# jianzhnie/ScaleRL

Hardware: NVIDIA H100
Metric: learner_frames_per_sec (higher is better)
Workload: dtype bf16

## Files before the change

### scalerl_b200/csrc/common.cuh

```cuda
#pragma once
#include <cuda_runtime.h>
#include <cuda_bf16.h>
#include <stdint.h>
#include "wgmma.cuh"

#define SRL_DEVINL __device__ __forceinline__

#ifndef SRL_SPIN_LIMIT
#define SRL_SPIN_LIMIT (1u << 24)
#endif

namespace srl {

SRL_DEVINL uint32_t smem_u32(const void* p) { return static_cast<uint32_t>(__cvta_generic_to_shared(p)); }

SRL_DEVINL void mbar_init(uint64_t* bar, uint32_t count) {
  asm volatile("mbarrier.init.shared::cta.b64 [%0], %1;" ::"r"(smem_u32(bar)), "r"(count) : "memory");
}
SRL_DEVINL void mbar_fence_init() { asm volatile("fence.mbarrier_init.release.cluster;" ::: "memory"); }
SRL_DEVINL void mbar_arrive(uint64_t* bar) {
  asm volatile("{\n\t.reg .b64 st;\n\tmbarrier.arrive.shared::cta.b64 st, [%0];\n\t}" ::"r"(smem_u32(bar)) : "memory");
}
SRL_DEVINL void mbar_arrive_expect_tx(uint64_t* bar, uint32_t bytes) {
  asm volatile("{\n\t.reg .b64 st;\n\tmbarrier.arrive.expect_tx.shared::cta.b64 st, [%0], %1;\n\t}" ::"r"(smem_u32(bar)), "r"(bytes)
// ... 111 lines not shown

SRL_DEVINL uint64_t make_smem_desc(uint32_t saddr, uint32_t lbo_bytes, uint32_t sbo_bytes) {
  uint64_t d = 0;
  d |= (uint64_t)((saddr & 0x3FFFF) >> 4);
  d |= (uint64_t)((lbo_bytes >> 4) & 0x3FFF) << 16;
  d |= (uint64_t)((sbo_bytes >> 4) & 0x3FFF) << 32;
  d |= (uint64_t)1 << 62;
  return d;
}
SRL_DEVINL uint64_t make_smem_desc_sw64(uint32_t saddr, uint32_t lbo_bytes, uint32_t sbo_bytes) {
  return (make_smem_desc(saddr, lbo_bytes, sbo_bytes) & ~((uint64_t)3 << 62)) | ((uint64_t)2 << 62);
}

SRL_DEVINL uint32_t swz128(uint32_t row, uint32_t chunk) { return row * 128u + ((chunk ^ (row & 7u)) << 4); }
SRL_DEVINL uint32_t swz64(uint32_t row, uint32_t chunk) { return row * 64u + ((chunk ^ ((row >> 1) & 3u)) << 4); }

SRL_DEVINL uint32_t pack_bf16x2(float lo, float hi) {
  __nv_bfloat162 v = __floats2bfloat162_rn(lo, hi);
  return *reinterpret_cast<uint32_t*>(&v);
}
SRL_DEVINL float bf16_lo(uint32_t v) { return __uint_as_float(v << 16); }
SRL_DEVINL float bf16_hi(uint32_t v) { return __uint_as_float(v & 0xFFFF0000u); }

SRL_DEVINL void red_add_v4(float* addr, float a, float b, float c, float d) {
  asm volatile("red.global.add.v4.f32 [%0], {%1, %2, %3, %4};" ::"l"(addr), "f"(a), "f"(b), "f"(c), "f"(d) : "memory");
}
SRL_DEVINL void red_add_16(float* dst, const float (&v)[16], float scale = 1.0f) {
#pragma unroll
  for (int j = 0; j < 16; j += 4) red_add_v4(dst + j, v[j] * scale, v[j + 1] * scale, v[j + 2] * scale, v[j + 3] * scale);
}

SRL_DEVINL int ld_action(const int64_t* p, int A) {
  const long long a = __ldg(reinterpret_cast<const long long*>(p));
  return a < 0 ? 0 : (a >= A ? A - 1 : (int)a);
}

SRL_DEVINL float warp_sum(float v) {
#pragma unroll
  for (int o = 16; o > 0; o >>= 1) v += __shfl_xor_sync(0xffffffffu, v, o);
  return v;
}

SRL_DEVINL bool take_ticket(float* scratch) {
  __threadfence();
  return atomicAdd(reinterpret_cast<unsigned*>(scratch), 1u) == gridDim.x - 1;
}
// ... 3 lines not shown
```

### scalerl_b200/csrc/encoder.cu

```cuda
#include "encoder_problems.cuh"
#include "tma_problems.cuh"
#include "res_problems.cuh"
#include "enc_fused.cuh"
#include "kernels.h"
#include <stdio.h>
#include <stdlib.h>

namespace srl {

constexpr int PACK_BLOCKS_FK = 256, PACK_BLOCKS_FD = 256, PACK_BLOCKS_CONV = 288;
SRL_DEVINL void pack_store(bf16* __restrict__ out, bf16* __restrict__ out_lo, int64_t i, float v) {
  const bf16 hi = __float2bfloat16_rn(v);
  out[i] = hi;
  if (out_lo) out_lo[i] = __float2bfloat16_rn(v - __bfloat162float(hi));
}
SRL_DEVINL void pack_store2(bf16* __restrict__ out, bf16* __restrict__ out_lo, int64_t i, float v0, float v1) {
  const bf16 h0 = __float2bfloat16_rn(v0), h1 = __float2bfloat16_rn(v1);
  *reinterpret_cast<uint32_t*>(out + i) = pack_bf16x2(v0, v1);
  if (out_lo) *reinterpret_cast<uint32_t*>(out_lo + i) = pack_bf16x2(v0 - __bfloat162float(h0), v1 - __bfloat162float(h1));
}
__global__ void __launch_bounds__(256) pack_weights_kernel(ParamPtrs p, bf16* __restrict__ out, bf16* __restrict__ out_lo, int skip_w1k) {
  pdl_wait(2);
  __shared__ __align__(16) float tile[64 * 99];
  const int t = threadIdx.x, b = blockIdx.x;
// ... 324 lines not shown
    static_assert(TFcFwd::SPLITS == FC_SPLITS, "split count");
    S.b(PS_FC_FWD);
    if (sp) SRL_TRY((igemm_tma_launch<TFcFwd, 1>(q, dim3(cdiv(frames, 128), 8 * FC_SPLITS), st)));
    else SRL_TRY((igemm_tma_launch<TFcFwd, 0>(q, dim3(cdiv(frames, 128), 8 * FC_SPLITS), st)));
    S.e(PS_FC_FWD); }
  return cudaSuccess;
}

cudaError_t encoder_backward(int frames, const EncoderBuffers& buf, const ParamPtrs& g, const TmaMaps& maps, int mode,
                             const StepStreams& S, BwdParts parts, bool a3t_done) {
  if (frames <= 0) return cudaSuccess;
  if ((mode != 0 && mode != 1) || !maps.valid) return cudaErrorInvalidValue;
  const int sp = mode;
  if (sp && !buf.lo.wpack) return cudaErrorInvalidValue;
  const bool do_fc = parts & BWD_FC, do_conv = parts & BWD_CONV;
  const cudaStream_t st = S.main, s1 = S.lane(LANE_FC_WGRAD), s2 = S.lane(LANE_CONV3_WGRAD), s3 = S.lane(LANE_CONV2_WGRAD);
  if (do_fc) {
    SRL_TRY(S.fork(LANE_FC_WGRAD));
    { const bool native = !sp && buf.a3t != nullptr;
      S.b(PS_FC_WGRAD);
      if (native) {
        if (!a3t_done) SRL_TRY(launch_a3_transpose(buf.hi.a3, buf.a3t, frames, s1));
        TFcWgradN::Params q{maps.hi.dhm64, maps.a3tm64, g.wf, g.bf, frames};
        SRL_TRY((igemm_tma_launch<TFcWgradN, 0>(q, dim3(1, 4 * (TFcWgradN::NCT + 1)), s1)));
      } else {
        TFcWgrad::Params q{maps.hi.dhm64, maps.hi.a3m64, maps.lo.dhm64, maps.lo.a3m64, g.wf, g.bf, frames};
        if (sp) SRL_TRY((igemm_tma_launch<TFcWgrad, 1>(q, dim3(1, 4 * 50), s1))); else SRL_TRY((igemm_tma_launch<TFcWgrad, 0>(q, dim3(1, 4 * 50), s1)));
      }
      S.e(PS_FC_WGRAD); }
    { TFcDgrad::Params q{maps.hi.dhm128, maps.hi.wfd, maps.lo.dhm128, maps.lo.wfd, buf.hi.a3, buf.hi.da3, buf.lo.da3, frames};
      S.b(PS_FC_DGRAD);
      if (sp) SRL_TRY((igemm_tma_launch<TFcDgrad, 1>(q, dim3(cdiv(frames, 128), 49), st))); else SRL_TRY((igemm_tma_launch<TFcDgrad, 0>(q, dim3(cdiv(frames, 128), 49), st)));
      S.e(PS_FC_DGRAD); }
    if (!do_conv) SRL_TRY(S.join(LANE_FC_WGRAD));
  }
  if (!do_conv) return cudaSuccess;
  SRL_TRY(S.fork(LANE_CONV3_WGRAD));
  float* part3 = buf.wgrad_part;
  float* part2 = part3 + (size_t)WG_PART_CTAS * WSP_W3;
  float* part1 = part2 + (size_t)WG_PART_CTAS * WSP_W2;
  int n3 = 0, n2 = 0, n1 = 0;
  { RConv3Wgrad::Params q{maps.hi.a2_w, maps.hi.da3g_b, maps.lo.a2_w, maps.lo.da3g_b, part3, frames * 81, 0};
    S.b(PS_CONV3_WGRAD); SRL_TRY(res_wgrad_launch<RConv3Wgrad>(q, side_wgrad_ctas(), s2, &n3, sp)); S.e(PS_CONV3_WGRAD); }
  if (!S.collapsed) SRL_TRY(launch_wgrad_reduce<WgradReduce3>(part3, n3, g.w3, g.b3, s2));
  { RConv3Dgrad::Params q{maps.hi.da3g_w, maps.hi.w3d, maps.lo.da3g_w, maps.lo.w3d, buf.hi.a2, buf.hi.da2, buf.lo.da2, frames};
    S.b(PS_CONV3_DGRAD); SRL_TRY(res_fwd_launch<RConv3Dgrad>(q, cdiv(frames * 81, 128), bwd_ctas(), st, sp)); S.e(PS_CONV3_DGRAD); }
  SRL_TRY(S.fork(LANE_CONV2_WGRAD));
// ... 22 lines not shown
```

### scalerl_b200/csrc/igemm_res.cuh

```cuda
#pragma once
#include "igemm_tma.cuh"

namespace srl {

constexpr int RES_THREADS = 384;
constexpr int RES_PRODUCER_REGS = 40, RES_CONSUMER_REGS = 232;
constexpr int RES_MAX_TAPS = 10;


template <int N, int ROWB, class F>
SRL_DEVINL void wg_acc_stage_bf16(const float (&d)[2][N / 2], uint8_t* buf, int wt, int bar, F f) {
  static_assert(ROWB % 16 == 0 && ROWB >= 2 * N, "16-byte aligned rows that hold N bf16");
  const int w = wt >> 5, l = wt & 31;
  named_bar(bar, 128);
#pragma unroll
  for (int h = 0; h < 2; ++h)
#pragma unroll
    for (int i = 0; i < N / 2; i += 2) {
      const int row = 64 * h + 16 * w + (l >> 2) + 8 * ((i >> 1) & 1), col = 8 * (i >> 2) + 2 * (l & 3);
      *reinterpret_cast<uint32_t*>(buf + row * ROWB + col * 2) = pack_bf16x2(f(col, d[h][i]), f(col + 1, d[h][i + 1]));
    }
  named_bar(bar, 128);
}
template <class P, int SPLIT>
struct ResFwdCfg {
  static constexpr int ALO = (SPLIT && P::A_LO) ? 1 : 0;
  static constexpr int WIN_BYTES = ((P::WROWS * 128 + 1023) / 1024) * 1024;
  static constexpr int IN_HI_BYTES = P::NWIN * WIN_BYTES;
  static constexpr int IN_BYTES = IN_HI_BYTES * (1 + ALO);
  static constexpr int W_HI_BYTES = P::NT * P::BN * 128;
  static constexpr int W_BYTES = W_HI_BYTES * (1 + SPLIT);
  static constexpr bool TILE_EPI = P::TILE_ROWB > 0 && !SPLIT;
  static constexpr int TILE_IMG_BYTES = 128 * P::TILE_ROWB > WG_IMG_BYTES ? 128 * P::TILE_ROWB : WG_IMG_BYTES;
  static constexpr bool IMG1 = !TILE_EPI && W_BYTES + IN_BYTES + 2 * WG_IMG_BYTES + 1024 + 256 > 232448;
  static constexpr int IMG_BYTES = TILE_EPI ? TILE_IMG_BYTES : IMG1 ? WG_IMG_BYTES / 2 : WG_IMG_BYTES;
  static constexpr int FIT = fit_stages(SPLIT ? P::SPLIT_STAGES : P::STAGES, W_BYTES + 2 * IMG_BYTES + 1024 + 256, IN_BYTES);
  static constexpr int STAGES = FIT > 1 ? FIT & ~1 : 1;
  static constexpr int SMEM_BYTES = W_BYTES + STAGES * IN_BYTES + 2 * IMG_BYTES + 1024 + 256;
  static_assert(SMEM_BYTES <= 232448, "shared memory budget (227 KB)");
  static_assert(W_BYTES % 1024 == 0, "weight block alignment");
  static_assert(P::BN == 32 || P::BN == 64 || P::BN == 128, "MMA N");
};

template <class P, int SPLIT>
__global__ void __launch_bounds__(RES_THREADS, 1) res_fwd_kernel(const __grid_constant__ typename P::Params p) {
  using C = ResFwdCfg<P, SPLIT>;
// ... 362 lines not shown
```

### scalerl_b200/csrc/igemm_tma.cuh

```cuda
#pragma once
#include <cuda.h>
#include "common.cuh"
#include "kernels.h"

namespace srl {

SRL_DEVINL void tma_prefetch_desc(const CUtensorMap* m) {
  asm volatile("prefetch.tensormap [%0];" ::"l"(reinterpret_cast<uint64_t>(m)) : "memory");
}
SRL_DEVINL void tma_load_2d(void* dst, const CUtensorMap* m, uint64_t* bar, int c0, int c1) {
  asm volatile("cp.async.bulk.tensor.2d.shared::cluster.global.mbarrier::complete_tx::bytes [%0], [%1, {%3, %4}], [%2];"
               ::"r"(smem_u32(dst)), "l"(reinterpret_cast<uint64_t>(m)), "r"(smem_u32(bar)), "r"(c0), "r"(c1) : "memory");
}
SRL_DEVINL void tma_load_3d(void* dst, const CUtensorMap* m, uint64_t* bar, int c0, int c1, int c2) {
  asm volatile("cp.async.bulk.tensor.3d.shared::cluster.global.mbarrier::complete_tx::bytes [%0], [%1, {%3, %4, %5}], [%2];"
               ::"r"(smem_u32(dst)), "l"(reinterpret_cast<uint64_t>(m)), "r"(smem_u32(bar)), "r"(c0), "r"(c1), "r"(c2) : "memory");
}
SRL_DEVINL void tma_load_4d(void* dst, const CUtensorMap* m, uint64_t* bar, int c0, int c1, int c2, int c3) {
  asm volatile("cp.async.bulk.tensor.4d.shared::cluster.global.mbarrier::complete_tx::bytes [%0], [%1, {%3, %4, %5, %6}], [%2];"
               ::"r"(smem_u32(dst)), "l"(reinterpret_cast<uint64_t>(m)), "r"(smem_u32(bar)), "r"(c0), "r"(c1), "r"(c2), "r"(c3)
               : "memory");
}
SRL_DEVINL void tma_load_5d(void* dst, const CUtensorMap* m, uint64_t* bar, int c0, int c1, int c2, int c3, int c4) {
  asm volatile("cp.async.bulk.tensor.5d.shared::cluster.global.mbarrier::complete_tx::bytes [%0], [%1, {%3, %4, %5, %6, %7}], [%2];"
               ::"r"(smem_u32(dst)), "l"(reinterpret_cast<uint64_t>(m)), "r"(smem_u32(bar)), "r"(c0), "r"(c1), "r"(c2), "r"(c3), "r"(c4)
               : "memory");
}

constexpr int IGT_THREADS = 288;

template <class P, int SPLIT = 0>
struct TmaCfg {
  static constexpr int KROWS = P::A_MN ? P::KROWS : 64;
  static constexpr int A_BYTES = P::A_MN ? 2 * KROWS * 128 : 128 * 128;
  static constexpr int B_BLOCKS = (P::BN + 63) / 64;
  static constexpr int B_BYTES = P::B_MN ? B_BLOCKS * KROWS * 128 : P::BN * 128;
  static constexpr int HALF_BYTES = A_BYTES + B_BYTES;
  static constexpr int STAGE_BYTES = HALF_BYTES * (1 + SPLIT);
  static constexpr int NB = P::BN / 2;
  static constexpr int STAGES = fit_stages(P::STAGES, 2 * WG_IMG_BYTES + 1024 + 256, STAGE_BYTES);
  static constexpr int SMEM_BYTES = STAGES * STAGE_BYTES + 2 * WG_IMG_BYTES + 1024 + 256;
  static_assert(SMEM_BYTES <= 232448, "shared memory budget (227 KB)");
  static_assert(NB == 32 || NB == 64 || NB == 128, "MMA N per warpgroup");
  static constexpr int MMAS = P::A_MN ? KROWS / 16 : 4;
  static_assert(A_BYTES % 1024 == 0 && B_BYTES % 1024 == 0, "operand tiles must keep 1024 B alignment (SWIZZLE_128B atoms)");
  static_assert(P::A_MN == P::B_MN, "mixed majors are not used");
  static_assert(KROWS % 16 == 0, "contraction rows per stage must be a multiple of MMA K = 16");
};

template <class P, int SPLIT>
SRL_DEVINL void igt_epilogue(const typename P::Params& p, int tm, int ty, int row, int c0, float (&v)[16]) {
  if constexpr (SPLIT) P::template epilogue16<1>(p, tm, ty, row, c0, v); else P::epilogue16(p, tm, ty, row, c0, v);
}
template <class P, int SPLIT>
SRL_DEVINL void igt_epilogue(const typename P::Params& p, int tm, int ty, int row, int c0, float (&v)[16], const uint4 (&pre)[2]) {
  if constexpr (SPLIT) P::template epilogue16<1>(p, tm, ty, row, c0, v, pre); else P::epilogue16(p, tm, ty, row, c0, v, pre);
}

template <class P, int SPLIT = 0>
__global__ void __launch_bounds__(IGT_THREADS) igemm_tma_kernel(const __grid_constant__ typename P::Params p) {
  using C = TmaCfg<P, SPLIT>;
  extern __shared__ uint8_t smem_raw[];
  uint8_t* smem = reinterpret_cast<uint8_t*>((reinterpret_cast<uintptr_t>(smem_raw) + 1023) & ~uintptr_t(1023));
  float* img = reinterpret_cast<float*>(smem + C::STAGES * C::STAGE_BYTES);
  uint64_t* bars = reinterpret_cast<uint64_t*>(smem + C::STAGES * C::STAGE_BYTES + 2 * WG_IMG_BYTES);
  uint64_t* full = bars;
  uint64_t* empty = bars + C::STAGES;

  const int tid = threadIdx.x;
  const int warp = tid >> 5;
  const int tm = blockIdx.x, ty = blockIdx.y;
  const int nkb = P::num_kblocks(p, tm, ty);

  if constexpr (P::ZERO_INIT) {
    if (P::zero_cta(ty)) {
      uint4* z = reinterpret_cast<uint4*>(smem);
      for (int i = tid; i < C::STAGES * C::STAGE_BYTES / 16; i += IGT_THREADS) z[i] = make_uint4(0, 0, 0, 0);
    }
    __syncthreads();
    for (int s = 0; s < C::STAGES; ++s) P::init_smem(p, tm, ty, smem + s * C::STAGE_BYTES, tid);
    fence_proxy_async_smem();
  }
  if (warp == 8 && (tid & 31) == 0) {
    for (int s = 0; s < C::STAGES; ++s) { mbar_init(&full[s], 1); mbar_init(&empty[s], 8); }
    mbar_fence_init();
    P::prefetch(p);
  }
  __syncthreads();
  pdl_wait(P::KID);
  if (tid == 256) pdl_launch();

  if (warp == 8) {
    const uint32_t leader = elect_one_sync();
    for (int kb = 0; kb < nkb; ++kb) {
      const int s = kb % C::STAGES;
      mbar_wait(&empty[s], ((kb / C::STAGES) & 1) ^ 1);
      if (leader) {
        uint8_t* sA = smem + s * C::STAGE_BYTES;
// ... 27 lines not shown
      wg_fence();
#pragma unroll
      for (int k = 0; k < C::MMAS; ++k) {
        const uint64_t ad = ad0 + (uint64_t)(k * ASTEP), bd = bd0 + (uint64_t)(k * BSTEP);
        wg_mma128<NB, P::A_MN ? 1 : 0, P::B_MN ? 1 : 0>(acc, ad, A_HI, bd, (kb | k) != 0);
        if constexpr (SPLIT) {
          wg_mma128<NB, P::A_MN ? 1 : 0, P::B_MN ? 1 : 0>(acc, ad, A_HI, bd + (uint64_t)(C::HALF_BYTES / 16), 1);
          wg_mma128<NB, P::A_MN ? 1 : 0, P::B_MN ? 1 : 0>(acc, ad + (uint64_t)(C::HALF_BYTES / 16), A_HI, bd, 1);
        }
      }
      wg_commit();
      if constexpr (C::STAGES > 1) {
        wg_wait_prev();
        __syncwarp();
        if (kb > 0 && (tid & 31) == 0) mbar_arrive(&empty[(kb - 1) % C::STAGES]);
      } else {
        wg_wait_all();
        __syncwarp();
        if ((tid & 31) == 0) mbar_arrive(&empty[s]);
      }
    }
    wg_wait_all();
    wg_fence_regs(acc[0]); wg_fence_regs(acc[1]);
    float* my_img = img + g * (WG_IMG_BYTES / 4);
#pragma unroll
    for (int c = 0; c < NB / 16; ++c) {
      float v[16];
      wg_acc_row16<NB>(acc, c, my_img, wt, 2 + g, v);
      if constexpr (P::PREFETCH) igt_epilogue<P, SPLIT>(p, tm, ty, wt, g * NB + c * 16, v, pre[c]);
      else igt_epilogue<P, SPLIT>(p, tm, ty, wt, g * NB + c * 16, v);
    }
  }
}

template <class P, int SPLIT = 0>
cudaError_t igemm_tma_launch(const typename P::Params& p, dim3 grid, cudaStream_t stream) {
  using C = TmaCfg<P, SPLIT>;
  if (grid.x == 0 || grid.y == 0) return cudaSuccess;
  static PerDeviceOnce once;
  { cudaError_t e = ensure_max_dynamic_smem(once, igemm_tma_kernel<P, SPLIT>, C::SMEM_BYTES); if (e != cudaSuccess) return e; }
  return launch_chain(igemm_tma_kernel<P, SPLIT>, grid, dim3(IGT_THREADS), C::SMEM_BYTES, stream, p);
}

}
```

### scalerl_b200/csrc/lstm.cu

```cuda
#include <new>
#include "tma_problems.cuh"
#include "kernels.h"
#include "errors.h"
#include "../../include/scalerl_b200.h"

namespace srl {

struct LGemmK {
  static constexpr int KID = 34;
  static constexpr bool PREFETCH = false;
  static constexpr int BN = 64, STAGES = 4, KROWS = 64;
  static constexpr bool A_MN = false, B_MN = false, ZERO_INIT = false;
  struct Params { SRL_TMAP a; SRL_TMAP b; float* C; int M, nkb, ldc, a_row0, c_row0; };
  SRL_DEVINL static void prefetch(const Params& p) { tma_prefetch_desc(&p.a); tma_prefetch_desc(&p.b); }
  SRL_DEVINL static int num_kblocks(const Params& p, int, int) { return p.nkb; }
  SRL_DEVINL static void issue(const Params& p, int tm, int ty, int kb, uint8_t* sA, uint8_t* sB, uint64_t* bar) {
    mbar_arrive_expect_tx(bar, 128 * 128 + 64 * 128);
    tma_load_2d(sA, &p.a, bar, kb * 64, p.a_row0 + tm * 128);
    tma_load_2d(sB, &p.b, bar, kb * 64, ty * 64);
  }
  SRL_DEVINL static void epilogue16(const Params& p, int tm, int ty, int row, int c0, float (&v)[16]) {
    const int m = tm * 128 + row;
    if (m >= p.M) return;
    float4* o = reinterpret_cast<float4*>(p.C + (size_t)(p.c_row0 + m) * p.ldc + ty * 64 + c0);
#pragma unroll
    for (int j = 0; j < 4; ++j) o[j] = make_float4(v[4 * j], v[4 * j + 1], v[4 * j + 2], v[4 * j + 3]);
  }
};
struct LGemmMN {
  static constexpr int KID = 35;
  static constexpr bool PREFETCH = false;
  static constexpr int BN = 64, STAGES = 4, KROWS = 64;
  static constexpr bool A_MN = true, B_MN = true, ZERO_INIT = false;
  struct Params { SRL_TMAP a; SRL_TMAP b; float* C; int R, ldc; };
  SRL_DEVINL static void prefetch(const Params& p) { tma_prefetch_desc(&p.a); tma_prefetch_desc(&p.b); }
  SRL_DEVINL static int num_kblocks(const Params& p, int, int) { return (p.R + 63) >> 6; }
  SRL_DEVINL static void init_smem(const Params&, int, int, uint8_t*, int, int) {}
  SRL_DEVINL static void issue(const Params& p, int tm, int ty, int kb, uint8_t* sA, uint8_t* sB, uint64_t* bar) {
    mbar_arrive_expect_tx(bar, 3 * 64 * 128);
    tma_load_2d(sA, &p.a, bar, tm * 128, kb * 64);
    tma_load_2d(sA + KROWS * 128, &p.a, bar, tm * 128 + 64, kb * 64);
    tma_load_2d(sB, &p.b, bar, ty * 64, kb * 64);
  }
  SRL_DEVINL static void epilogue16(const Params& p, int tm, int ty, int row, int c0, float (&v)[16]) {
    float4* o = reinterpret_cast<float4*>(p.C + (size_t)(tm * 128 + row) * p.ldc + ty * 64 + c0);
#pragma unroll
    for (int j = 0; j < 4; ++j) o[j] = make_float4(v[4 * j], v[4 * j + 1], v[4 * j + 2], v[4 * j + 3]);
  }
};

SRL_DEVINL float sigmoidf_(float x) { return 1.0f / (1.0f + expf(-x)); }

__global__ void lstm_pad_bf16_kernel(const float* __restrict__ x, int rows, int H, int Hp, __nv_bfloat16* __restrict__ out) {
  const int64_t i = (int64_t)blockIdx.x * blockDim.x + threadIdx.x;
  if (i >= (int64_t)rows * Hp) return;
  const int r = (int)(i / Hp), j = (int)(i - (int64_t)r * Hp);
// ... 658 lines not shown
```

### scalerl_b200/csrc/res_problems.cuh

```cuda
#pragma once
#include "igemm_res.cuh"
#include "encoder_problems.cuh"

namespace srl {

template <int SPLIT>
SRL_DEVINL void store_act16(bf16* hi, bf16* lo, size_t elem_off, const float (&v)[16]) {
  store_bf16x16(hi + elem_off, v);
  if constexpr (SPLIT) {
    float r[16];
#pragma unroll
    for (int j = 0; j < 16; ++j) r[j] = v[j] - __bfloat162float(__float2bfloat16_rn(v[j]));
    store_bf16x16(lo + elem_off, r);
  }
}

struct RConv1Fwd {
  static constexpr int KID = 11;
  static constexpr int BN = 32, NT = 4, NWIN = 1, WROWS = 128 + 22, STAGES = 4, SPLIT_STAGES = 4;
  static constexpr bool A_LO = false;
  struct Params { SRL_TMAP in0; SRL_TMAP w; SRL_TMAP w_lo; const float* bias; bf16* out; bf16* out_lo; int NF; int NFS; };
  static constexpr bool W_AFTER_WAIT = true;
  SRL_DEVINL static void prefetch(const Params& p) { tma_prefetch_desc(&p.in0); tma_prefetch_desc(&p.w); }
  SRL_DEVINL static int num_tiles(const Params& p) { return (p.NF * 441 + 127) >> 7; }
  SRL_DEVINL static constexpr int tap_win(int) { return 0; }
  SRL_DEVINL static constexpr int tap_shift(int j) { return (j >> 1) * 21 + (j & 1); }
  SRL_DEVINL static void load_windows(const Params& p, int t, uint8_t* dst, int, uint64_t* bar, bool) { tma_load_2d(dst, &p.in0, bar, 0, t * 128); }
  SRL_DEVINL static void prefetch16(const Params&, int, int, int, uint4 (&)[2]) {}
  static constexpr int TILE_ROWB = 80;
  SRL_DEVINL static void prefetch_tile(const Params&, int, int, uint4 (&)[BN / 16][2]) {}
  SRL_DEVINL static void epilogue_tile(const Params& p, int t, int wt, const float (&acc)[2][BN / 2], uint8_t* img, int bar,
                                       const uint4 (&)[BN / 16][2]) {
    wg_acc_stage_bf16<BN, TILE_ROWB>(acc, img, wt, bar, [&](int c, float v) { return fmaxf(fmaf(v, 1.0f / 255.0f, __ldg(p.bias + c)), 0.f); });
#pragma unroll
    for (int s = 0; s < 4; ++s) {
      const int e = s * 128 + wt, q = e >> 2, k = e & 3;
      const int Q = t * 128 + q, n = Q / 441, r = Q - n * 441, oh = r / 21, ow = r - oh * 21;
      if (n >= p.NF || oh >= 20 || ow >= 20) continue;
      const size_t prow = (size_t)(oh & 1) * p.NFS * 100 + (size_t)n * 100 + (oh >> 1) * 10 + (ow >> 1);
      *reinterpret_cast<uint4*>(p.out + prow * 64 + (ow & 1) * 32 + k * 8) = *reinterpret_cast<const uint4*>(img + q * TILE_ROWB + k * 16);
    }
  }
  template <int SPLIT>
  SRL_DEVINL static void epilogue16(const Params& p, int t, int row, int c0, float (&v)[16], const uint4 (&)[2]) {
    const int Q = t * 128 + row, n = Q / 441, r = Q - n * 441, oh = r / 21, ow = r - oh * 21;
    if (n >= p.NF || oh >= 20 || ow >= 20) return;
#pragma unroll
    for (int j = 0; j < 16; ++j) v[j] = fmaxf(fmaf(v[j], 1.0f / 255.0f, __ldg(p.bias + c0 + j)), 0.f);
    const size_t prow = (size_t)(oh & 1) * p.NFS * 100 + (size_t)n * 100 + (oh >> 1) * 10 + (ow >> 1);
    store_act16<SPLIT>(p.out, p.out_lo, prow * 64 + (ow & 1) * 32 + c0, v);
  }
};

struct RConv2Fwd {
  static constexpr int KID = 12;
  static constexpr bool W_AFTER_WAIT = false;
// ... 73 lines not shown
  static constexpr bool W_AFTER_WAIT = false;
  static constexpr int BN = 128, NT = 4, NWIN = 1, WROWS = 128 + 11, STAGES = 3, SPLIT_STAGES = 2;
  static constexpr bool A_LO = true;
  struct Params { SRL_TMAP in0; SRL_TMAP w; SRL_TMAP in0_lo; SRL_TMAP w_lo; const bf16* act; bf16* dx; bf16* dx_lo; int NB; int NF; };
  SRL_DEVINL static void prefetch(const Params& p) { tma_prefetch_desc(&p.in0); tma_prefetch_desc(&p.w); }
  SRL_DEVINL static int num_tiles(const Params& p) { return (p.NB * 100 + 127) >> 7; }
  SRL_DEVINL static constexpr int tap_win(int) { return 0; }
  SRL_DEVINL static constexpr int tap_shift(int j) { return 11 - ((j >> 1) * 10 + (j & 1)); }
  SRL_DEVINL static void load_windows(const Params& p, int t, uint8_t* dst, int, uint64_t* bar, bool lo) { tma_load_2d(dst, lo ? &p.in0_lo : &p.in0, bar, 0, t * 128 - 11); }
  SRL_DEVINL static void prefetch16(const Params& p, int t, int row, int c0, uint4 (&m)[2]) {
    const int Q = t * 128 + row, cls = c0 >> 5, c = c0 & 31;
    if (Q < p.NB * 100) ld_mask16(p.act + ((size_t)(cls >> 1) * p.NF * 100 + Q) * 64 + (cls & 1) * 32 + c, m);
  }
  static constexpr int TILE_ROWB = 272;
  SRL_DEVINL static void prefetch_tile(const Params& p, int t, int wt, uint4 (&m)[BN / 16][2]) {
#pragma unroll
    for (int s = 0; s < 16; ++s) {
      const int e = s * 128 + wt, ph = e >> 10, Q = t * 128 + ((e >> 3) & 127);
      if (Q < p.NB * 100) m[s >> 1][s & 1] = ldg16(p.act + ((size_t)ph * p.NF * 100 + Q) * 64 + (e & 7) * 8);
    }
  }
  SRL_DEVINL static void epilogue_tile(const Params& p, int t, int wt, const float (&acc)[2][BN / 2], uint8_t* img, int bar,
                                       const uint4 (&m)[BN / 16][2]) {
    wg_acc_stage_bf16<BN, TILE_ROWB>(acc, img, wt, bar, [](int, float v) { return v; });
#pragma unroll
    for (int s = 0; s < 16; ++s) {
      const int e = s * 128 + wt, ph = e >> 10, q = (e >> 3) & 127, k = e & 7;
      const int Q = t * 128 + q, n = Q / 100, r = Q - n * 100, i = r / 10, j = r - i * 10;
      if (n >= p.NB) continue;
      const uint4 x = *reinterpret_cast<const uint4*>(img + q * TILE_ROWB + ph * 128 + k * 16), mk = m[s >> 1][s & 1];
      *reinterpret_cast<uint4*>(p.dx + ((size_t)n * 441 + (2 * i + ph) * 21 + 2 * j) * 32 + k * 8) =
          make_uint4(relu_mask_bf16x2(x.x, mk.x), relu_mask_bf16x2(x.y, mk.y), relu_mask_bf16x2(x.z, mk.z), relu_mask_bf16x2(x.w, mk.w));
    }
  }
  template <int SPLIT>
  SRL_DEVINL static void epilogue16(const Params& p, int t, int row, int c0, float (&v)[16], const uint4 (&m)[2]) {
    const int Q = t * 128 + row, n = Q / 100, r = Q - n * 100, i = r / 10, j = r - i * 10;
    if (n >= p.NB) return;
    const int cls = c0 >> 5, c = c0 & 31, ph = cls >> 1, pw = cls & 1;
    relu_mask16_pre(m, v);
    store_act16<SPLIT>(p.dx, p.dx_lo, ((size_t)n * 441 + (2 * i + ph) * 21 + 2 * j + pw) * 32 + c, v);
  }
};

struct RConv3Wgrad {
  static constexpr int KID = 21;
  static constexpr int NBLK = 9, CWG = 3, NWIN = 1, WROWS = 128 + 20, STAGES = 3, SPLIT_STAGES = 2;
// ... 45 lines not shown
```

### scalerl_b200/csrc/tma_problems.cuh

```cuda
#pragma once
#include "igemm_tma.cuh"
#include "encoder_problems.cuh"

namespace srl {

#define SRL_TMAP alignas(64) CUtensorMap

struct TFcFwd {
  static constexpr int KID = 31;
  static constexpr bool PREFETCH = false;
  static constexpr int BN = 64, STAGES = 4, SPLITS = 4;
  static constexpr bool A_MN = false, B_MN = false, ZERO_INIT = false;
  static constexpr int KROWS = 64;
  struct Params { SRL_TMAP a3m; SRL_TMAP w; SRL_TMAP a3m_lo; SRL_TMAP w_lo; float* out; int M; };
  SRL_DEVINL static void prefetch(const Params& p) { tma_prefetch_desc(&p.a3m); tma_prefetch_desc(&p.w); }
  SRL_DEVINL static int kb_begin(int split) { return (49 * split) / SPLITS; }
  SRL_DEVINL static void issue_split(const Params& p, int tm, int ty, int kb, uint8_t* st, int a_bytes, int half, uint64_t* bar) {
    const int k = (kb_begin(ty % SPLITS) + kb) * 64;
    mbar_arrive_expect_tx(bar, 2 * (128 * 128 + 64 * 128));
    tma_load_2d(st, &p.a3m, bar, k, tm * 128);
    tma_load_2d(st + a_bytes, &p.w, bar, k, (ty / SPLITS) * 64);
    tma_load_2d(st + half, &p.a3m_lo, bar, k, tm * 128);
    tma_load_2d(st + half + a_bytes, &p.w_lo, bar, k, (ty / SPLITS) * 64);
  }
  template <int SPLIT>
  SRL_DEVINL static void epilogue16(const Params& p, int tm, int ty, int row, int c0, float (&v)[16]) { epilogue16(p, tm, ty, row, c0, v); }
  SRL_DEVINL static int num_kblocks(const Params&, int, int ty) { const int sp = ty % SPLITS; return kb_begin(sp + 1) - kb_begin(sp); }
  SRL_DEVINL static void issue(const Params& p, int tm, int ty, int kb, uint8_t* sA, uint8_t* sB, uint64_t* bar) {
    const int k = (kb_begin(ty % SPLITS) + kb) * 64;
    mbar_arrive_expect_tx(bar, 128 * 128 + 64 * 128);
    tma_load_2d(sA, &p.a3m, bar, k, tm * 128);
    tma_load_2d(sB, &p.w, bar, k, (ty / SPLITS) * 64);
  }
  SRL_DEVINL static void epilogue16(const Params& p, int tm, int ty, int row, int c0, float (&v)[16]) {
    const int m = tm * 128 + row;
    if (m >= p.M) return;
    float4* o = reinterpret_cast<float4*>(p.out + ((size_t)(ty % SPLITS) * p.M + m) * 512 + (ty / SPLITS) * 64 + c0);
#pragma unroll
    for (int j = 0; j < 4; ++j) o[j] = make_float4(v[4 * j], v[4 * j + 1], v[4 * j + 2], v[4 * j + 3]);
  }
};

struct TFcDgrad {
  static constexpr int KID = 32;
  static constexpr bool PREFETCH = true;
  static constexpr int BN = 64, STAGES = 4;
  static constexpr bool A_MN = false, B_MN = false, ZERO_INIT = false;
  static constexpr int KROWS = 64;
  struct Params { SRL_TMAP dhm; SRL_TMAP w; SRL_TMAP dhm_lo; SRL_TMAP w_lo; const bf16* a3; bf16* da3; bf16* da3_lo; int M; };
  SRL_DEVINL static void prefetch(const Params& p) { tma_prefetch_desc(&p.dhm); tma_prefetch_desc(&p.w); }
  SRL_DEVINL static int num_kblocks(const Params&, int, int) { return 8; }
  SRL_DEVINL static void issue_split(const Params& p, int tm, int ty, int kb, uint8_t* st, int a_bytes, int half, uint64_t* bar) {
    mbar_arrive_expect_tx(bar, 2 * (128 * 128 + 64 * 128));
    tma_load_2d(st, &p.dhm, bar, kb * 64, tm * 128);
    tma_load_2d(st + a_bytes, &p.w, bar, kb * 64, ty * 64);
    tma_load_2d(st + half, &p.dhm_lo, bar, kb * 64, tm * 128);
    tma_load_2d(st + half + a_bytes, &p.w_lo, bar, kb * 64, ty * 64);
  }
  SRL_DEVINL static void issue(const Params& p, int tm, int ty, int kb, uint8_t* sA, uint8_t* sB, uint64_t* bar) {
    mbar_arrive_expect_tx(bar, 128 * 128 + 64 * 128);
    tma_load_2d(sA, &p.dhm, bar, kb * 64, tm * 128);
    tma_load_2d(sB, &p.w, bar, kb * 64, ty * 64);
  }
  SRL_DEVINL static void prefetch16(const Params& p, int tm, int ty, int row, int c0, uint4 (&mk)[2]) {
    const int m = tm * 128 + row;
    if (m < p.M) ld_mask16(p.a3 + (size_t)m * 3136 + ty * 64 + c0, mk);
  }
  SRL_DEVINL static void epilogue16(const Params& p, int tm, int ty, int row, int c0, float (&v)[16], const uint4 (&mk)[2]) {
    epilogue16<0>(p, tm, ty, row, c0, v, mk);
  }
// ... 2 lines not shown
    const int m = tm * 128 + row;
    if (m >= p.M) return;
    relu_mask16_pre(mk, v);
    const size_t o = ((size_t)m * 81 + (ty / 7) * 9 + ty % 7) * 64 + c0;
    store_bf16x16(p.da3 + o, v);
    if constexpr (SPLIT) {
      float r[16];
#pragma unroll
      for (int j = 0; j < 16; ++j) r[j] = v[j] - __bfloat162float(__float2bfloat16_rn(v[j]));
      store_bf16x16(p.da3_lo + o, r);
    }
  }
};

SRL_DEVINL void fill_ones(uint8_t* dst, int bytes, int tid) {
  uint4* q = reinterpret_cast<uint4*>(dst);
  for (int i = tid; i < bytes / 16; i += IGT_THREADS) q[i] = make_uint4(0x3F803F80u, 0x3F803F80u, 0x3F803F80u, 0x3F803F80u);
}

struct TFcWgrad {
  static constexpr int KID = 33;
  static constexpr bool PREFETCH = false;
  static constexpr int BN = 64, STAGES = 4, KROWS = 64;
  static constexpr bool A_MN = true, B_MN = true, ZERO_INIT = true;
  struct Params { SRL_TMAP dhm; SRL_TMAP a3m; SRL_TMAP dhm_lo; SRL_TMAP a3m_lo; float* dw; float* db; int M; };
  SRL_DEVINL static void prefetch(const Params& p) { tma_prefetch_desc(&p.dhm); tma_prefetch_desc(&p.a3m); }
  SRL_DEVINL static void issue_split(const Params& p, int, int ty, int kb, uint8_t* st, int a_bytes, int half, uint64_t* bar) {
    const int hw = ty >> 2, j0 = (ty & 3) * 128;
    mbar_arrive_expect_tx(bar, (hw < 49 ? 6 : 4) * 64 * 128);
    tma_load_2d(st, &p.dhm, bar, j0, kb * 64);
    tma_load_2d(st + KROWS * 128, &p.dhm, bar, j0 + 64, kb * 64);
    tma_load_2d(st + half, &p.dhm_lo, bar, j0, kb * 64);
    tma_load_2d(st + half + KROWS * 128, &p.dhm_lo, bar, j0 + 64, kb * 64);
    if (hw < 49) {
      tma_load_2d(st + a_bytes, &p.a3m, bar, hw * 64, kb * 64);
      tma_load_2d(st + half + a_bytes, &p.a3m_lo, bar, hw * 64, kb * 64);
    }
  }
  template <int SPLIT>
  SRL_DEVINL static void epilogue16(const Params& p, int tm, int ty, int row, int c0, float (&v)[16]) { epilogue16(p, tm, ty, row, c0, v); }
  SRL_DEVINL static bool zero_cta(int) { return true; }
  SRL_DEVINL static int num_kblocks(const Params& p, int, int) { return (p.M + 63) >> 6; }
  SRL_DEVINL static void init_smem(const Params&, int, int ty, uint8_t* stage, int tid) {
    if ((ty >> 2) == 49) fill_ones(stage + 2 * KROWS * 128, KROWS * 128, tid);
  }
  SRL_DEVINL static void issue(const Params& p, int, int ty, int kb, uint8_t* sA, uint8_t* sB, uint64_t* bar) {
    const int hw = ty >> 2, j0 = (ty & 3) * 128;
    mbar_arrive_expect_tx(bar, (hw < 49 ? 3 : 2) * 64 * 128);
    tma_load_2d(sA, &p.dhm, bar, j0, kb * 64);
    tma_load_2d(sA + KROWS * 128, &p.dhm, bar, j0 + 64, kb * 64);
    if (hw < 49) tma_load_2d(sB, &p.a3m, bar, hw * 64, kb * 64);
  }
  SRL_DEVINL static void epilogue16(const Params& p, int, int ty, int row, int c0, float (&v)[16]) {
    const int j = (ty & 3) * 128 + row, hw = ty >> 2;
    if (hw < 49) {
#pragma unroll
      for (int jj = 0; jj < 16; ++jj) p.dw[(size_t)j * 3136 + (c0 + jj) * 49 + hw] = v[jj];
    } else if (c0 == 0) {
      p.db[j] = v[0];
    }
  }
};

struct TFcWgradN {
  static constexpr int KID = 36;
  static constexpr bool PREFETCH = false;
  static constexpr int BN = 256, STAGES = 4, KROWS = 64, NCT = 13;
  static constexpr bool A_MN = true, B_MN = true, ZERO_INIT = true;
  struct Params { SRL_TMAP dhm; SRL_TMAP a3tm; float* dw; float* db; int M; };
  SRL_DEVINL static void prefetch(const Params& p) { tma_prefetch_desc(&p.dhm); tma_prefetch_desc(&p.a3tm); }
  SRL_DEVINL static bool zero_cta(int ty) { return (ty >> 2) == NCT; }
  SRL_DEVINL static int num_kblocks(const Params& p, int, int) { return (p.M + 63) >> 6; }
  SRL_DEVINL static void init_smem(const Params&, int, int ty, uint8_t* stage, int tid) {
    if ((ty >> 2) == NCT) fill_ones(stage + 2 * KROWS * 128, KROWS * 128, tid);
  }
  SRL_DEVINL static void issue(const Params& p, int, int ty, int kb, uint8_t* sA, uint8_t* sB, uint64_t* bar) {
    const int ct = ty >> 2, j0 = (ty & 3) * 128;
    const int nb = ct < NCT ? (ct == NCT - 1 ? 1 : 4) : 0;
    mbar_arrive_expect_tx(bar, (2 + nb) * 64 * 128);
    tma_load_2d(sA, &p.dhm, bar, j0, kb * 64);
    tma_load_2d(sA + KROWS * 128, &p.dhm, bar, j0 + 64, kb * 64);
    for (int q = 0; q < nb; ++q) tma_load_2d(sB + q * KROWS * 128, &p.a3tm, bar, ct * 256 + q * 64, kb * 64);
  }
  SRL_DEVINL static void epilogue16(const Params& p, int, int ty, int row, int c0, float (&v)[16]) {
    const int j = (ty & 3) * 128 + row, ct = ty >> 2, col = ct * 256 + c0;
    if (ct < NCT) {
      if (col < 3136) {
        float4* d = reinterpret_cast<float4*>(p.dw + (size_t)j * 3136 + col);
#pragma unroll
        for (int q = 0; q < 4; ++q) d[q] = make_float4(v[4 * q], v[4 * q + 1], v[4 * q + 2], v[4 * q + 3]);
      }
    } else if (c0 == 0) {
      p.db[j] = v[0];
    }
  }
};

}
```

Measured before the change: 2.483 million.

## Fold FC wgrad bias into last column tile and stage epilogue through ring

```diff
diff --git a/scalerl_b200/csrc/common.cuh b/scalerl_b200/csrc/common.cuh
--- a/scalerl_b200/csrc/common.cuh
+++ b/scalerl_b200/csrc/common.cuh
@@ -157,6 +157,24 @@
 SRL_DEVINL float bf16_lo(uint32_t v) { return __uint_as_float(v << 16); }
 SRL_DEVINL float bf16_hi(uint32_t v) { return __uint_as_float(v & 0xFFFF0000u); }
 
+template <int N, int ROWB, class T, class F>
+SRL_DEVINL void wg_acc_stage(const float (&d)[2][N / 2], uint8_t* buf, int wt, int bar, F f) {
+  static_assert(ROWB % 16 == 0 && ROWB >= (int)sizeof(T) * N, "16-byte aligned rows that hold N values");
+  const int w = wt >> 5, l = wt & 31;
+  named_bar(bar, 128);
+#pragma unroll
+  for (int h = 0; h < 2; ++h)
+#pragma unroll
+    for (int i = 0; i < N / 2; i += 2) {
+      const int row = 64 * h + 16 * w + (l >> 2) + 8 * ((i >> 1) & 1), col = 8 * (i >> 2) + 2 * (l & 3);
+      if constexpr (sizeof(T) == 2)
+        *reinterpret_cast<uint32_t*>(buf + row * ROWB + col * 2) = pack_bf16x2(f(col, d[h][i]), f(col + 1, d[h][i + 1]));
+      else
+        *reinterpret_cast<float2*>(buf + row * ROWB + col * 4) = make_float2(f(col, d[h][i]), f(col + 1, d[h][i + 1]));
+    }
+  named_bar(bar, 128);
+}
+
 SRL_DEVINL void red_add_v4(float* addr, float a, float b, float c, float d) {
   asm volatile("red.global.add.v4.f32 [%0], {%1, %2, %3, %4};" ::"l"(addr), "f"(a), "f"(b), "f"(c), "f"(d) : "memory");
 }
diff --git a/scalerl_b200/csrc/encoder.cu b/scalerl_b200/csrc/encoder.cu
--- a/scalerl_b200/csrc/encoder.cu
+++ b/scalerl_b200/csrc/encoder.cu
@@ -370,7 +370,7 @@
       if (native) {
         if (!a3t_done) SRL_TRY(launch_a3_transpose(buf.hi.a3, buf.a3t, frames, s1));
         TFcWgradN::Params q{maps.hi.dhm64, maps.a3tm64, g.wf, g.bf, frames};
-        SRL_TRY((igemm_tma_launch<TFcWgradN, 0>(q, dim3(1, 4 * (TFcWgradN::NCT + 1)), s1)));
+        SRL_TRY((igemm_tma_launch<TFcWgradN, 0>(q, dim3(1, 4 * TFcWgradN::NCT), s1)));
       } else {
         TFcWgrad::Params q{maps.hi.dhm64, maps.hi.a3m64, maps.lo.dhm64, maps.lo.a3m64, g.wf, g.bf, frames};
         if (sp) SRL_TRY((igemm_tma_launch<TFcWgrad, 1>(q, dim3(1, 4 * 50), s1))); else SRL_TRY((igemm_tma_launch<TFcWgrad, 0>(q, dim3(1, 4 * 50), s1)));
diff --git a/scalerl_b200/csrc/igemm_res.cuh b/scalerl_b200/csrc/igemm_res.cuh
--- a/scalerl_b200/csrc/igemm_res.cuh
+++ b/scalerl_b200/csrc/igemm_res.cuh
@@ -8,20 +8,6 @@
 constexpr int RES_MAX_TAPS = 10;
 
 
-template <int N, int ROWB, class F>
-SRL_DEVINL void wg_acc_stage_bf16(const float (&d)[2][N / 2], uint8_t* buf, int wt, int bar, F f) {
-  static_assert(ROWB % 16 == 0 && ROWB >= 2 * N, "16-byte aligned rows that hold N bf16");
-  const int w = wt >> 5, l = wt & 31;
-  named_bar(bar, 128);
-#pragma unroll
-  for (int h = 0; h < 2; ++h)
-#pragma unroll
-    for (int i = 0; i < N / 2; i += 2) {
-      const int row = 64 * h + 16 * w + (l >> 2) + 8 * ((i >> 1) & 1), col = 8 * (i >> 2) + 2 * (l & 3);
-      *reinterpret_cast<uint32_t*>(buf + row * ROWB + col * 2) = pack_bf16x2(f(col, d[h][i]), f(col + 1, d[h][i + 1]));
-    }
-  named_bar(bar, 128);
-}
 template <class P, int SPLIT>
 struct ResFwdCfg {
   static constexpr int ALO = (SPLIT && P::A_LO) ? 1 : 0;
diff --git a/scalerl_b200/csrc/igemm_tma.cuh b/scalerl_b200/csrc/igemm_tma.cuh
--- a/scalerl_b200/csrc/igemm_tma.cuh
+++ b/scalerl_b200/csrc/igemm_tma.cuh
@@ -38,9 +38,12 @@
   static constexpr int HALF_BYTES = A_BYTES + B_BYTES;
   static constexpr int STAGE_BYTES = HALF_BYTES * (1 + SPLIT);
   static constexpr int NB = P::BN / 2;
-  static constexpr int STAGES = fit_stages(P::STAGES, 2 * WG_IMG_BYTES + 1024 + 256, STAGE_BYTES);
-  static constexpr int SMEM_BYTES = STAGES * STAGE_BYTES + 2 * WG_IMG_BYTES + 1024 + 256;
+  static constexpr bool TILE_EPI = P::TILE_ROWB > 0 && !SPLIT;
+  static constexpr int IMG_BYTES = TILE_EPI ? 0 : 2 * WG_IMG_BYTES;
+  static constexpr int STAGES = fit_stages(P::STAGES, IMG_BYTES + 1024 + 256, STAGE_BYTES);
+  static constexpr int SMEM_BYTES = STAGES * STAGE_BYTES + IMG_BYTES + 1024 + 256;
   static_assert(SMEM_BYTES <= 232448, "shared memory budget (227 KB)");
+  static_assert(!TILE_EPI || 2 * 128 * P::TILE_ROWB <= STAGES * STAGE_BYTES, "both warpgroups' tile images fit the stage ring");
   static_assert(NB == 32 || NB == 64 || NB == 128, "MMA N per warpgroup");
   static constexpr int MMAS = P::A_MN ? KROWS / 16 : 4;
   static_assert(A_BYTES % 1024 == 0 && B_BYTES % 1024 == 0, "operand tiles must keep 1024 B alignment (SWIZZLE_128B atoms)");
@@ -63,7 +66,7 @@
   extern __shared__ uint8_t smem_raw[];
   uint8_t* smem = reinterpret_cast<uint8_t*>((reinterpret_cast<uintptr_t>(smem_raw) + 1023) & ~uintptr_t(1023));
   float* img = reinterpret_cast<float*>(smem + C::STAGES * C::STAGE_BYTES);
-  uint64_t* bars = reinterpret_cast<uint64_t*>(smem + C::STAGES * C::STAGE_BYTES + 2 * WG_IMG_BYTES);
+  uint64_t* bars = reinterpret_cast<uint64_t*>(smem + C::STAGES * C::STAGE_BYTES + C::IMG_BYTES);
   uint64_t* full = bars;
   uint64_t* empty = bars + C::STAGES;
 
@@ -73,7 +76,7 @@
   const int nkb = P::num_kblocks(p, tm, ty);
 
   if constexpr (P::ZERO_INIT) {
-    if (P::zero_cta(ty)) {
+    if constexpr (P::ZERO_RING) {
       uint4* z = reinterpret_cast<uint4*>(smem);
       for (int i = tid; i < C::STAGES * C::STAGE_BYTES / 16; i += IGT_THREADS) z[i] = make_uint4(0, 0, 0, 0);
     }
@@ -147,13 +150,20 @@
     }
     wg_wait_all();
     wg_fence_regs(acc[0]); wg_fence_regs(acc[1]);
-    float* my_img = img + g * (WG_IMG_BYTES / 4);
+    if constexpr (C::TILE_EPI) {
+      named_bar(1, 256);
+      uint8_t* my_tile = smem + g * 128 * P::TILE_ROWB;
+      wg_acc_stage<NB, P::TILE_ROWB, float>(acc, my_tile, wt, 2 + g, [](int, float v) { return v; });
+      P::epilogue_tile(p, tm, ty, g, wt, my_tile);
+    } else {
+      float* my_img = img + g * (WG_IMG_BYTES / 4);
 #pragma unroll
-    for (int c = 0; c < NB / 16; ++c) {
-      float v[16];
-      wg_acc_row16<NB>(acc, c, my_img, wt, 2 + g, v);
-      if constexpr (P::PREFETCH) igt_epilogue<P, SPLIT>(p, tm, ty, wt, g * NB + c * 16, v, pre[c]);
-      else igt_epilogue<P, SPLIT>(p, tm, ty, wt, g * NB + c * 16, v);
+      for (int c = 0; c < NB / 16; ++c) {
+        float v[16];
+        wg_acc_row16<NB>(acc, c, my_img, wt, 2 + g, v);
+        if constexpr (P::PREFETCH) igt_epilogue<P, SPLIT>(p, tm, ty, wt, g * NB + c * 16, v, pre[c]);
+        else igt_epilogue<P, SPLIT>(p, tm, ty, wt, g * NB + c * 16, v);
+      }
     }
   }
 }
diff --git a/scalerl_b200/csrc/lstm.cu b/scalerl_b200/csrc/lstm.cu
--- a/scalerl_b200/csrc/lstm.cu
+++ b/scalerl_b200/csrc/lstm.cu
@@ -11,6 +11,7 @@
   static constexpr bool PREFETCH = false;
   static constexpr int BN = 64, STAGES = 4, KROWS = 64;
   static constexpr bool A_MN = false, B_MN = false, ZERO_INIT = false;
+  static constexpr int TILE_ROWB = 0;
   struct Params { SRL_TMAP a; SRL_TMAP b; float* C; int M, nkb, ldc, a_row0, c_row0; };
   SRL_DEVINL static void prefetch(const Params& p) { tma_prefetch_desc(&p.a); tma_prefetch_desc(&p.b); }
   SRL_DEVINL static int num_kblocks(const Params& p, int, int) { return p.nkb; }
@@ -32,6 +33,7 @@
   static constexpr bool PREFETCH = false;
   static constexpr int BN = 64, STAGES = 4, KROWS = 64;
   static constexpr bool A_MN = true, B_MN = true, ZERO_INIT = false;
+  static constexpr int TILE_ROWB = 0;
   struct Params { SRL_TMAP a; SRL_TMAP b; float* C; int R, ldc; };
   SRL_DEVINL static void prefetch(const Params& p) { tma_prefetch_desc(&p.a); tma_prefetch_desc(&p.b); }
   SRL_DEVINL static int num_kblocks(const Params& p, int, int) { return (p.R + 63) >> 6; }
diff --git a/scalerl_b200/csrc/res_problems.cuh b/scalerl_b200/csrc/res_problems.cuh
--- a/scalerl_b200/csrc/res_problems.cuh
+++ b/scalerl_b200/csrc/res_problems.cuh
@@ -31,7 +31,7 @@
   SRL_DEVINL static void prefetch_tile(const Params&, int, int, uint4 (&)[BN / 16][2]) {}
   SRL_DEVINL static void epilogue_tile(const Params& p, int t, int wt, const float (&acc)[2][BN / 2], uint8_t* img, int bar,
                                        const uint4 (&)[BN / 16][2]) {
-    wg_acc_stage_bf16<BN, TILE_ROWB>(acc, img, wt, bar, [&](int c, float v) { return fmaxf(fmaf(v, 1.0f / 255.0f, __ldg(p.bias + c)), 0.f); });
+    wg_acc_stage<BN, TILE_ROWB, bf16>(acc, img, wt, bar, [&](int c, float v) { return fmaxf(fmaf(v, 1.0f / 255.0f, __ldg(p.bias + c)), 0.f); });
 #pragma unroll
     for (int s = 0; s < 4; ++s) {
       const int e = s * 128 + wt, q = e >> 2, k = e & 3;
@@ -151,7 +151,7 @@
   }
   SRL_DEVINL static void epilogue_tile(const Params& p, int t, int wt, const float (&acc)[2][BN / 2], uint8_t* img, int bar,
                                        const uint4 (&m)[BN / 16][2]) {
-    wg_acc_stage_bf16<BN, TILE_ROWB>(acc, img, wt, bar, [](int, float v) { return v; });
+    wg_acc_stage<BN, TILE_ROWB, bf16>(acc, img, wt, bar, [](int, float v) { return v; });
 #pragma unroll
     for (int s = 0; s < 16; ++s) {
       const int e = s * 128 + wt, ph = e >> 10, q = (e >> 3) & 127, k = e & 7;
diff --git a/scalerl_b200/csrc/tma_problems.cuh b/scalerl_b200/csrc/tma_problems.cuh
--- a/scalerl_b200/csrc/tma_problems.cuh
+++ b/scalerl_b200/csrc/tma_problems.cuh
@@ -11,6 +11,7 @@
   static constexpr bool PREFETCH = false;
   static constexpr int BN = 64, STAGES = 4, SPLITS = 4;
   static constexpr bool A_MN = false, B_MN = false, ZERO_INIT = false;
+  static constexpr int TILE_ROWB = 0;
   static constexpr int KROWS = 64;
   struct Params { SRL_TMAP a3m; SRL_TMAP w; SRL_TMAP a3m_lo; SRL_TMAP w_lo; float* out; int M; };
   SRL_DEVINL static void prefetch(const Params& p) { tma_prefetch_desc(&p.a3m); tma_prefetch_desc(&p.w); }
@@ -46,6 +47,7 @@
   static constexpr bool PREFETCH = true;
   static constexpr int BN = 64, STAGES = 4;
   static constexpr bool A_MN = false, B_MN = false, ZERO_INIT = false;
+  static constexpr int TILE_ROWB = 0;
   static constexpr int KROWS = 64;
   struct Params { SRL_TMAP dhm; SRL_TMAP w; SRL_TMAP dhm_lo; SRL_TMAP w_lo; const bf16* a3; bf16* da3; bf16* da3_lo; int M; };
   SRL_DEVINL static void prefetch(const Params& p) { tma_prefetch_desc(&p.dhm); tma_prefetch_desc(&p.w); }
@@ -94,7 +96,8 @@
   static constexpr int KID = 33;
   static constexpr bool PREFETCH = false;
   static constexpr int BN = 64, STAGES = 4, KROWS = 64;
-  static constexpr bool A_MN = true, B_MN = true, ZERO_INIT = true;
+  static constexpr bool A_MN = true, B_MN = true, ZERO_INIT = true, ZERO_RING = true;
+  static constexpr int TILE_ROWB = 0;
   struct Params { SRL_TMAP dhm; SRL_TMAP a3m; SRL_TMAP dhm_lo; SRL_TMAP a3m_lo; float* dw; float* db; int M; };
   SRL_DEVINL static void prefetch(const Params& p) { tma_prefetch_desc(&p.dhm); tma_prefetch_desc(&p.a3m); }
   SRL_DEVINL static void issue_split(const Params& p, int, int ty, int kb, uint8_t* st, int a_bytes, int half, uint64_t* bar) {
@@ -111,7 +114,6 @@
   }
   template <int SPLIT>
   SRL_DEVINL static void epilogue16(const Params& p, int tm, int ty, int row, int c0, float (&v)[16]) { epilogue16(p, tm, ty, row, c0, v); }
-  SRL_DEVINL static bool zero_cta(int) { return true; }
   SRL_DEVINL static int num_kblocks(const Params& p, int, int) { return (p.M + 63) >> 6; }
   SRL_DEVINL static void init_smem(const Params&, int, int ty, uint8_t* stage, int tid) {
     if ((ty >> 2) == 49) fill_ones(stage + 2 * KROWS * 128, KROWS * 128, tid);
@@ -138,32 +140,36 @@
   static constexpr int KID = 36;
   static constexpr bool PREFETCH = false;
   static constexpr int BN = 256, STAGES = 4, KROWS = 64, NCT = 13;
-  static constexpr bool A_MN = true, B_MN = true, ZERO_INIT = true;
+  static constexpr bool A_MN = true, B_MN = true, ZERO_INIT = true, ZERO_RING = false;
+  static constexpr int TILE_ROWB = (BN / 2) * 4 + 32;
   struct Params { SRL_TMAP dhm; SRL_TMAP a3tm; float* dw; float* db; int M; };
   SRL_DEVINL static void prefetch(const Params& p) { tma_prefetch_desc(&p.dhm); tma_prefetch_desc(&p.a3tm); }
-  SRL_DEVINL static bool zero_cta(int ty) { return (ty >> 2) == NCT; }
   SRL_DEVINL static int num_kblocks(const Params& p, int, int) { return (p.M + 63) >> 6; }
   SRL_DEVINL static void init_smem(const Params&, int, int ty, uint8_t* stage, int tid) {
-    if ((ty >> 2) == NCT) fill_ones(stage + 2 * KROWS * 128, KROWS * 128, tid);
+    if ((ty >> 2) == NCT - 1) fill_ones(stage + 3 * KROWS * 128, KROWS * 128, tid);
   }
   SRL_DEVINL static void issue(const Params& p, int, int ty, int kb, uint8_t* sA, uint8_t* sB, uint64_t* bar) {
     const int ct = ty >> 2, j0 = (ty & 3) * 128;
-    const int nb = ct < NCT ? (ct == NCT - 1 ? 1 : 4) : 0;
+    const int nb = ct == NCT - 1 ? 1 : 4;
     mbar_arrive_expect_tx(bar, (2 + nb) * 64 * 128);
     tma_load_2d(sA, &p.dhm, bar, j0, kb * 64);
     tma_load_2d(sA + KROWS * 128, &p.dhm, bar, j0 + 64, kb * 64);
     for (int q = 0; q < nb; ++q) tma_load_2d(sB + q * KROWS * 128, &p.a3tm, bar, ct * 256 + q * 64, kb * 64);
   }
-  SRL_DEVINL static void epilogue16(const Params& p, int, int ty, int row, int c0, float (&v)[16]) {
-    const int j = (ty & 3) * 128 + row, ct = ty >> 2, col = ct * 256 + c0;
-    if (ct < NCT) {
-      if (col < 3136) {
-        float4* d = reinterpret_cast<float4*>(p.dw + (size_t)j * 3136 + col);
+  SRL_DEVINL static void epilogue_tile(const Params& p, int, int ty, int g, int wt, const uint8_t* img) {
+    const int ct = ty >> 2, j0 = (ty & 3) * 128, col = ct * 256 + g * 128, w = wt >> 5, l = wt & 31;
+    if (col >= 3136) return;
+    if (ct == NCT - 1) p.db[j0 + wt] = *reinterpret_cast<const float*>(img + wt * TILE_ROWB + 64 * 4);
+    if (4 * l >= 3136 - col) return;
+    const uint32_t src = smem_u32(img) + l * 16;
+    float* dst = p.dw + (size_t)j0 * 3136 + col + 4 * l;
 #pragma unroll
-        for (int q = 0; q < 4; ++q) d[q] = make_float4(v[4 * q], v[4 * q + 1], v[4 * q + 2], v[4 * q + 3]);
-      }
-    } else if (c0 == 0) {
-      p.db[j] = v[0];
+    for (int r0 = w; r0 < 128; r0 += 32) {
+      uint4 v[8];
+#pragma unroll
+      for (int i = 0; i < 8; ++i) v[i] = lds128(src + (r0 + 4 * i) * TILE_ROWB);
+#pragma unroll
+      for (int i = 0; i < 8; ++i) *reinterpret_cast<uint4*>(dst + (size_t)(r0 + 4 * i) * 3136) = v[i];
     }
   }
 };
```

After: 2.511 million, median of 6. No clear change (+1.1%).
